# gillett-hernandez/rust-pathtracer

Hardware: AMD Instinct MI355X
Metric: Msamples/s (paths×spp/s) Cornell box 1024², max_bounces=8; 1/2/4/8 GPU (higher is better)
Workload: dtype f32

## Files before the change

### include/pt_api.h

```cpp
#ifndef PT_API_H
#define PT_API_H

#include <stddef.h>
#include <stdint.h>

#ifdef __cplusplus
extern "C" {
#endif

typedef int32_t pt_status;
enum {
    PT_OK = 0,
    PT_ERR_INVALID_ARGUMENT = 1,
    PT_ERR_NO_DEVICE = 2,
    PT_ERR_OUT_OF_MEMORY = 3,
    PT_ERR_UNSUPPORTED = 4,
    PT_ERR_DEVICE = 5
};

enum { PT_TAG_MATERIAL = 0, PT_TAG_LIGHT = 1, PT_TAG_CAMERA = 2 };
#define PT_MATERIAL_ID(tag, index) ((((uint32_t)(tag)) << 16) | ((uint32_t)(index) & 0xffffu))
#define PT_MATERIAL_TAG(id) (((id) >> 16) & 0x3u)
#define PT_MATERIAL_INDEX(id) ((id) & 0xffffu)
#define PT_MATERIAL_NONE 0xffffffffu
// ... 147 lines not shown
    uint32_t medium_aware;
} pt_render_desc;

enum {
    PT_TUNE_NO_LDS = 1u << 0,
    PT_TUNE_NO_CORE_LDS = 1u << 1,
    PT_TUNE_NO_PARK = 1u << 2,
    PT_TUNE_NO_LIVE_LIST = 1u << 3,
    PT_TUNE_EXACT_SLAB = 1u << 4,
    PT_TUNE_NO_CULL = 1u << 5,
    PT_TUNE_NO_SWEEP = 1u << 6,
    PT_TUNE_NO_MESH_SWEEP = 1u << 7,
    PT_TUNE_NO_KNOWN_LIGHT = 1u << 8,
    PT_TUNE_GENERAL_FORMS = 1u << 9,
    PT_TUNE_NO_FUSE = 1u << 10,
    PT_TUNE_NO_STAGE_TIMING = 1u << 11,
    PT_TUNE_MULTI_RCCL = 1u << 12,
    PT_TUNE_NO_ONE_LIGHT = 1u << 14,
    PT_TUNE_NO_CONVEX = 1u << 15,
    PT_TUNE_NO_MESH_SHORTCUTS = 1u << 16,
    PT_TUNE_NO_AXIS_SCAN = 1u << 13,
    PT_TUNE_NO_PASS_OVERLAP = 1u << 17,
    PT_TUNE_PASS_SKEW_SHIFT = 18,
    PT_TUNE_PASS_SKEW_MASK = 7
};
typedef struct pt_tuning {
    uint32_t flags;
    uint32_t batch_slots;
    uint32_t blocks_per_cu;
    uint32_t park_blocks_per_cu;
    int32_t park_dynamic;
    uint32_t shade_form;
    uint32_t lds_all_limit;
    uint32_t multi_virtual;
    uint32_t walk_evict_below;
    uint32_t walk_search_below;
    uint32_t park_block;
    uint32_t light_prepass_max;
    uint32_t top_evict_below;
    uint32_t group_evict_below;
    uint32_t reserved[2];
} pt_tuning;
void pt_tuning_default(pt_tuning* tuning);

typedef struct pt_profile {
    uint64_t bounce_rays, shadow_rays, light_rays, camera_rays, env_hits;
    double seconds;
// ... 73 lines not shown
```

### rust-pathtracer_amd/api.py

```python
import ctypes as C
import numpy as np

PT_OK = 0
PT_ERR_INVALID_ARGUMENT = 1
PT_ERR_UNSUPPORTED = 4
TAG_MATERIAL, TAG_LIGHT, TAG_CAMERA = 0, 1, 2
MATERIAL_NONE = 0xFFFFFFFF

CURVE_LINEAR, CURVE_TABULATED, CURVE_CAUCHY, CURVE_EXPONENTIAL, CURVE_INV_EXPONENTIAL, CURVE_BLACKBODY, CURVE_CONST = range(7)
INTERP_LINEAR, INTERP_NEAREST, INTERP_CUBIC = range(3)
TEXTURE1, TEXTURE4 = 1, 4
MATERIAL_LAMBERTIAN, MATERIAL_GGX, MATERIAL_DIFFUSE_LIGHT, MATERIAL_SHARP_LIGHT, MATERIAL_PASSTHROUGH = range(5)
MEDIUM_HG, MEDIUM_RAYLEIGH = range(2)
SIDED_FORWARD, SIDED_REVERSE, SIDED_DUAL = range(3)
SHAPE_RECT, SHAPE_SPHERE, SHAPE_DISK, SHAPE_MESH = range(4)
AXIS_X, AXIS_Y, AXIS_Z = range(3)
ENV_CONSTANT, ENV_SUN, ENV_HDR = range(3)


def material_id(tag, index):
    return ((tag & 3) << 16) | (index & 0xFFFF)


class Curve(C.Structure):
# ... 123 lines not shown
class ResidentDenoiseDesc(C.Structure):
    _fields_ = [("filter", DenoiseDesc), ("flags", C.c_uint32), ("reserved", C.c_uint32 * 3)]


class GuideChainDesc(C.Structure):
    _fields_ = [("max_chain", C.c_uint32), ("alpha_max", C.c_float), ("reserved", C.c_uint32 * 2)]


class Profile(C.Structure):
    _fields_ = [("bounce_rays", C.c_uint64), ("shadow_rays", C.c_uint64), ("light_rays", C.c_uint64),
                ("camera_rays", C.c_uint64), ("env_hits", C.c_uint64), ("seconds", C.c_double),
                ("kernel_seconds", C.c_double * 8), ("kernel_launches", C.c_uint64 * 8), ("stage_items", C.c_uint64 * 8)]

    def as_dict(self):
        return {"bounce_rays": self.bounce_rays, "shadow_rays": self.shadow_rays, "light_rays": self.light_rays,
                "camera_rays": self.camera_rays, "env_hits": self.env_hits, "seconds": self.seconds,
                "kernel_seconds": list(self.kernel_seconds), "kernel_launches": list(self.kernel_launches), "stage_items": list(self.stage_items)}


TUNE_NO_LDS, TUNE_NO_CORE_LDS, TUNE_NO_PARK, TUNE_NO_LIVE_LIST, TUNE_EXACT_SLAB, TUNE_NO_CULL, TUNE_NO_SWEEP, TUNE_NO_MESH_SWEEP, TUNE_NO_KNOWN_LIGHT, \
    TUNE_GENERAL_FORMS, TUNE_NO_FUSE, TUNE_NO_STAGE_TIMING, TUNE_MULTI_RCCL, TUNE_NO_AXIS_SCAN, TUNE_NO_ONE_LIGHT, TUNE_NO_CONVEX, TUNE_NO_MESH_SHORTCUTS, \
    TUNE_NO_PASS_OVERLAP = (1 << i for i in range(18))
TUNE_PASS_SKEW_SHIFT, TUNE_PASS_SKEW_MASK = 18, 7


class Tuning(C.Structure):
    _fields_ = [("flags", C.c_uint32), ("batch_slots", C.c_uint32), ("blocks_per_cu", C.c_uint32), ("park_blocks_per_cu", C.c_uint32),
                ("park_dynamic", C.c_int32), ("shade_form", C.c_uint32), ("lds_all_limit", C.c_uint32), ("multi_virtual", C.c_uint32),
                ("walk_evict_below", C.c_uint32), ("walk_search_below", C.c_uint32), ("park_block", C.c_uint32), ("light_prepass_max", C.c_uint32), ("top_evict_below", C.c_uint32), ("group_evict_below", C.c_uint32), ("reserved", C.c_uint32 * 2)]


class OutputDesc(C.Structure):
    _fields_ = [("width", C.c_uint32), ("height", C.c_uint32), ("tonemap", C.c_int32), ("luminance_only", C.c_int32),
                ("exposure", C.c_float), ("key_value", C.c_float), ("white_point", C.c_float), ("colorspace", C.c_int32),
                ("factor", C.c_float)]


TONEMAP_CLAMP, TONEMAP_REINHARD0, TONEMAP_REINHARD1 = range(3)
COLORSPACE_SRGB, COLORSPACE_REC709, COLORSPACE_REC2020 = range(3)
COMPARE_ABSOLUTE, COMPARE_RMSE, COMPARE_RELATIVE = range(3)


class CompareStats(C.Structure):
    _fields_ = [("linf", C.c_double * 4), ("mean_abs", C.c_double * 4), ("rmse", C.c_double), ("pixel_min", C.c_float),
                ("pixel_max", C.c_float), ("nonfinite", C.c_uint64)]

# ... 366 lines not shown
        handle = C.c_void_p()
        if tuning is not None:
            if library._scene_create_tuned is None:
                raise PtError(PT_ERR_UNSUPPORTED, "this library does not export %sscene_create_tuned (pt_tuning is the HIP engine's)" % library.prefix)
            library.check(library._scene_create_tuned(C.byref(desc), C.byref(tuning), C.byref(handle)))
        else:
            library.check(library._scene_create(C.byref(desc), C.byref(handle)))
        self.handle = handle

    def close(self):
        if self.handle:
            self.library._scene_destroy(self.handle)
            self.handle = None

    def __del__(self):
        try:
            self.close()
        except Exception:
            pass

    def uses_leaf_sweep(self):
        return bool(self.library._debug_scene_info(self.handle, 4))

    def render(self, rd):
        film = np.zeros((rd.height, rd.width, 4), dtype=np.float32)
        prof = Profile()
        self.library.check(self.library._render(self.handle, C.byref(rd), _fp(film), C.byref(prof)))
        return film, prof

    def render_spectral(self, rd, bins):
        if self.library._render_spectral is None:
            raise PtError(PT_ERR_UNSUPPORTED, "%s has no %srender_spectral entry" % (self.library.path, self.library.prefix))
        film = np.zeros((rd.height, rd.width, 4), dtype=np.float32)
        spectral = np.zeros((max(int(bins), 0), rd.height, rd.width), dtype=np.float32)
        sd = SpectralDesc(bins)
        prof = Profile()
        self.library.check(self.library._render_spectral(self.handle, C.byref(rd), C.byref(sd), _fp(film), _fp(spectral), C.byref(prof)))
        return film, spectral, prof

    def render_spectral_multi(self, rd, bins, device_mask=0):
        if self.library._render_spectral_multi is None:
            raise PtError(PT_ERR_UNSUPPORTED, "%s has no %srender_spectral_multi entry" % (self.library.path, self.library.prefix))
        film = np.zeros((rd.height, rd.width, 4), dtype=np.float32)
        spectral = np.zeros((max(int(bins), 0), rd.height, rd.width), dtype=np.float32)
        sd = SpectralDesc(bins)
        prof = Profile()
# ... 370 lines not shown
```

### rust-pathtracer_amd/csrc/pt_engine.hip

```cpp
#include <hip/hip_runtime.h>

#include <dlfcn.h>
#include <rccl/rccl.h>

#include <algorithm>
#include <chrono>
#include <condition_variable>
#include <functional>
#include <mutex>
#include <thread>
#include <cstdio>
#include <cstring>
#include <string>
#include <vector>

#include "pt_kernels.h"
#include "../../include/pt_adaptive.h"
#include "../../include/pt_spectral.h"
#include "../../include/pt_api.h"
#include "../../include/pt_debug.h"
#include "../../include/pt_denoise.h"
#include "../../include/pt_light_groups.h"
#include "pt_adaptive_select.h"
#include "pt_light_groups_launch.h"
// ... 256 lines not shown
    const float* film = nullptr; const uint32_t* counts = nullptr; const double* stats = nullptr; const float* spectral = nullptr;
    const float* denoised_bins = nullptr;
    GrowBuf load_film, load_counts, load_stats, load_spectral;
    GrowBuf guides, albedo, bin_albedo;
    GrowBuf color[2], geo, tent, flags, grad, bin_buf[2];
    GrowBuf den_film, den_var, den_bins;
    void end() { parts = 0; width = height = bins = 0; }
    void tidy() {
        if (!(parts & (PT_RESIDENT_BINS | PT_RESIDENT_BIN_ALBEDO | PT_RESIDENT_DENOISED_BINS))) bins = 0;
        if (!parts) width = height = 0;
    }
    struct pt_resident_info info() const { struct pt_resident_info i; i.width = width; i.height = height; i.bins = bins; i.parts = parts; return i; }
};

struct pt_scene {
    pth::HostScene host;
    pt_tuning tuning;
    MultiSetup multi;
    uint32_t* d_blob = nullptr;
    float* d_tex = nullptr;
    uint32_t blob_words = 0;
    int lds_mode = 0;
    uint32_t lacks = 0;
    int device = 0, num_cus = 0;
    DeviceBuffers buf;
    DeviceBuffers buf2;
    hipStream_t pass_stream = nullptr;
    std::vector<hipEvent_t> pass_deps;
    AdaptiveBuffers adaptive;
    std::vector<hipEvent_t> events, events2;
    GrowBuf film_cache;
    GrowBuf spectral_cache;
    bool spectral_valid = false;
    uint32_t spectral_width = 0, spectral_height = 0, spectral_bins = 0;
    std::vector<pt_scene*> spectral_shards;
    std::vector<uint32_t> shard_px;
    GrowBuf shard_packed;
    bool groups_valid = false;
    uint32_t groups_width = 0, groups_height = 0, groups_count = 0;
    GrowBuf group_films_cache, group_table, group_mix_cache;
    ResidentSet resident;
    GrowBuf assemble_staging, assemble_px;
    GrowBuf project_cache;
    std::vector<pt_scene*> replicas;
};

// ... 247 lines not shown
        if (sweep) for (uint32_t j = 0; j < bl[PT_HDR_SWEEP_COUNT]; ++j) walked += (bl[bl[PT_HDR_SWEEP_OFF] + j * PT_SWEEP_INST_WORDS + 1] & PT_SWEEP_WALKED) ? 1u : 0u;
        if (parked && walked == 1u) group_evict = tn.group_evict_below ? tn.group_evict_below : kGroupEvictBelow;
    }
    cfg.walk_policy = (tn.walk_evict_below ? tn.walk_evict_below : kWalkEvictBelow) | (tn.walk_search_below ? tn.walk_search_below : kWalkSearchBelow) << 8
                    | ((tn.flags & PT_TUNE_NO_AXIS_SCAN) ? 0u : PT_WALK_SCAN_AXIS)
                    | (top_evict <= 1u ? 0u : top_evict << 24)
                    | (group_evict <= 1u ? 0u : group_evict << 17);
    float env_prob; std::memcpy(&env_prob, &sc->host.blob[PT_HDR_ENV_PROB], sizeof env_prob);
    bool has_ggx = false;
    for (uint32_t i = 0; i < sc->host.blob[PT_HDR_MATERIAL_COUNT]; ++i) {
        const uint32_t kind = sc->host.blob[sc->host.blob[PT_HDR_MATERIAL_OFF] + i * PT_MAT_WORDS + PT_MAT_KIND];
        has_ggx = has_ggx || kind == PT_MATERIAL_GGX || kind == PT_MATERIAL_PASSTHROUGH;
    }
    const bool certs = !rd.medium_aware && (sc->host.blob[PT_HDR_FLAGS] & PT_FLAG_CONVEX) != 0u;
    const int shade_form = rd.medium_aware ? PT_SHADE_MEDIUM
                         : (env_prob != 0.0f || tn.shade_form == 2 || grouped) ? PT_SHADE_FULL : (has_ggx || certs || tn.shade_form == 1) ? PT_SHADE_NO_ENV : PT_SHADE_LEAN;
    cfg.certs = certs;
    uint32_t live_list = ((trav_form == PT_FORM_SWEEP || trav_form == PT_FORM_WALK || trav_form == PT_FORM_ANY) && shade_form == PT_SHADE_LEAN && !(tn.flags & PT_TUNE_NO_LIVE_LIST)) ? 1u : 0u;
#ifdef PT_EXPERIMENTS
    if (cfg.live_lists || getenv("PT_AMD_EXP_SHADOW")) live_list = 0u;
#endif
    const uint32_t camera_record = (shade_form == PT_SHADE_LEAN || shade_form == PT_SHADE_FULL || shade_form == PT_SHADE_MEDIUM) ? 1u : 0u;
    cfg.fuse = !(tn.flags & PT_TUNE_NO_FUSE) && (!hero || PT_FUSE_HERO) && trav_form == PT_FORM_SWEEP && shade_form == PT_SHADE_LEAN && (cfg.lacks & PT_SCENE_NO_XF) != 0;
    const uint32_t path_fields = hero ? Layout<4>::path_fields : (rd.medium_aware ? (uint32_t)PS_FIELDS + 2u : Layout<1>::path_fields);
    const uint32_t item_fields = hero ? Layout<4>::shadow_queue_fields(rd.light_samples ? rd.light_samples : 1) : Layout<1>::shadow_queue_fields(rd.light_samples ? rd.light_samples : 1);
    *plan = RenderPlan{capacity, grid, hero, park_block, park_block_extend, trav_form, shade_form, park_dynamic, park_big, cfg, live_list, camera_record,
                       path_fields, item_fields};
    return PT_OK;
}

pt_status read_profile(pt_scene* sc, const RenderPlan& plan, bool second_set, uint64_t camera_rays, uint64_t accumulated_pixels, const double* stage_ms, const uint64_t* stage_launches,
                       uint32_t rounds, double seconds, pt_profile* profile) {
    memset(profile, 0, sizeof(*profile));
    std::vector<unsigned long long> bs((size_t)plan.grid * BS_FIELDS);
    unsigned long long c[BS_FIELDS] = {0, 0, 0, 0, 0, 0};
    for (const unsigned long long* d_bs : {(const unsigned long long*)sc->buf.block_stats, (const unsigned long long*)(second_set ? sc->buf2.block_stats : nullptr)}) {
        if (!d_bs) continue;
        HIP_TRY(hipMemcpy(bs.data(), d_bs, sizeof(unsigned long long) * bs.size(), hipMemcpyDeviceToHost));
        for (int g = 0; g < plan.grid; ++g) for (int k = 0; k < BS_FIELDS; ++k) c[k] += bs[(size_t)g * BS_FIELDS + k];
    }
    profile->camera_rays = camera_rays;
    profile->bounce_rays = c[BS_VERTICES] + camera_rays;
    profile->shadow_rays = c[BS_SHADOW_RAYS];
    profile->env_hits = c[BS_ENV_HITS];
    profile->seconds = seconds;
    for (int i = 0; i < ST_COUNT; ++i) { profile->kernel_seconds[i] = stage_ms[i] * 1e-3; profile->kernel_launches[i] = stage_launches[i]; }
// ... 2 lines not shown
    profile->stage_items[6] = (uint64_t)plan.cfg.park_block;
    profile->stage_items[7] = plan.camera_record;
    profile->stage_items[5] = c[BS_MEDIUM_DROPS];
    profile->kernel_launches[5] = rounds;
    return PT_OK;
}

enum { DEP_FORK = 0, DEP_ACCUMULATED = 1, DEP_SKEW = 3, DEP_COUNT = 5 };

pt_status render_impl(pt_scene* sc, const pt_render_desc* rdp, float* d_film, hipStream_t stream, pt_profile* profile, const RenderJob& job) {
    if (!sc || !rdp || !d_film) return fail(PT_ERR_INVALID_ARGUMENT, "null argument");
    pt_render_desc rd;
    std::string err;
    if (!pth::normalize_render_desc(*rdp, (uint32_t)sc->host.cameras.size(), &rd, &err)) return fail(PT_ERR_INVALID_ARGUMENT, err);
    HIP_TRY(hipSetDevice(sc->device));

    const pt_adaptive_desc* adaptive = job.adaptive;
    std::vector<uint32_t> own_list;
    if (!job.shard_list) own_list = pth::shard_pixels(rd.width, rd.height, rd.tile_width, rd.tile_height, rd.shard_index, rd.shard_count);
    const std::vector<uint32_t>& pixels = job.shard_list ? *job.shard_list : own_list;
    RenderPlan plan;
    pt_status st = plan_render(sc, rd, job, pixels, stream, &plan);
    if (st != PT_OK) return st;
    const uint32_t capacity = plan.capacity;
    const int grid = plan.grid, trav_form = plan.trav_form, shade_form = plan.shade_form;
    const bool hero = plan.hero, park_dynamic = plan.park_dynamic;
    LaunchCfg cfg = plan.cfg;

#ifdef PT_EXPERIMENTS
    const bool need_hits = true;
#else
    const bool need_hits = !cfg.fuse;
#endif
    const uint32_t group_count = job.groups ? job.groups->group_count : 0u;
    st = ensure_buffers(sc, sc->buf, capacity, rd.light_samples, pixels.size() ? pixels.size() : 1, grid, (hero || rd.medium_aware) ? 4u : 1u, plan.park_block, need_hits, group_count);
    if (st != PT_OK) return st;
    DeviceBuffers& b = sc->buf;
    bool overlap = !(sc->tuning.flags & PT_TUNE_NO_PASS_OVERLAP);
    if (overlap) {
        const uint32_t n_px = (uint32_t)pixels.size();
        overlap = pth::plan_passes(n_px, rd.first_sample, adaptive ? rd.spp : rd.sample_count, capacity, rd.phase_samples).size() >= 2
               || (adaptive && adaptive->max_samples > rd.spp && pth::plan_passes(n_px, rd.spp, adaptive->step < adaptive->max_samples - rd.spp ? adaptive->step : adaptive->max_samples - rd.spp, capacity, rd.phase_samples).size() >= 2);
    }
    if (overlap) {
        bool ok = ensure_buffers(sc, sc->buf2, capacity, rd.light_samples, 0, grid, (hero || rd.medium_aware) ? 4u : 1u, plan.park_block, need_hits, group_count) == PT_OK;
        if (ok && !sc->pass_stream) ok = hipStreamCreateWithFlags(&sc->pass_stream, hipStreamNonBlocking) == hipSuccess;
// ... 255 lines not shown
    if (e == hipSuccess) e = hipMemcpy(sc->d_tex, sc->host.tex.data(), sizeof(float) * sc->host.tex.size(), hipMemcpyHostToDevice);
    if (e != hipSuccess) return fail(e == hipErrorOutOfMemory ? PT_ERR_OUT_OF_MEMORY : PT_ERR_DEVICE, hipGetErrorString(e));
    if (sc->lds_mode != PT_LDS_NONE) {
        e = allow_lds_extend(kParkBlobLimitBytes);
        if (e == hipSuccess) e = allow_lds_shade(kLdsBlobLimitBytes > PT_SHADE_LDS_BUDGET ? kLdsBlobLimitBytes : PT_SHADE_LDS_BUDGET);
        if (e == hipSuccess) e = allow_lds_shadow(kParkBlobLimitBytes + 16u * (64u * PT_MAX_LIGHT_SAMPLES + 64u) * 4u);
        if (e == hipSuccess) e = allow_lds_groups(kLdsBlobLimitBytes > PT_SHADE_LDS_BUDGET ? kLdsBlobLimitBytes : PT_SHADE_LDS_BUDGET, kLdsBlobLimitBytes);
        if (e != hipSuccess) return fail(PT_ERR_DEVICE, std::string("hipFuncSetAttribute(MaxDynamicSharedMemorySize): ") + hipGetErrorString(e));
    }
    return PT_OK;
}

void pt_tuning_default(pt_tuning* t) {
    if (!t) return;
    memset(t, 0, sizeof(*t));
    const struct { const char* name; uint32_t bit; } flags[] = {
        {"PT_AMD_NO_LDS", PT_TUNE_NO_LDS}, {"PT_AMD_NO_CORE_LDS", PT_TUNE_NO_CORE_LDS}, {"PT_AMD_NO_PARK", PT_TUNE_NO_PARK},
#ifdef PT_EXPERIMENTS
        {"PT_AMD_POOL", PT_TUNE_EXPERIMENT_POOL},
#endif

        {"PT_AMD_EXACT_SLAB", PT_TUNE_EXACT_SLAB}, {"PT_AMD_NO_CULL", PT_TUNE_NO_CULL}, {"PT_AMD_NO_SWEEP", PT_TUNE_NO_SWEEP}, {"PT_AMD_NO_MESH_SWEEP", PT_TUNE_NO_MESH_SWEEP},
        {"PT_AMD_NO_KNOWN_LIGHT", PT_TUNE_NO_KNOWN_LIGHT}, {"PT_AMD_GENERAL_FORMS", PT_TUNE_GENERAL_FORMS}, {"PT_AMD_NO_FUSE", PT_TUNE_NO_FUSE}, {"PT_AMD_MULTI_RCCL", PT_TUNE_MULTI_RCCL}, {"PT_AMD_NO_AXIS_SCAN", PT_TUNE_NO_AXIS_SCAN}, {"PT_AMD_NO_ONE_LIGHT", PT_TUNE_NO_ONE_LIGHT}, {"PT_AMD_NO_CONVEX", PT_TUNE_NO_CONVEX}, {"PT_AMD_NO_MESH_SHORTCUTS", PT_TUNE_NO_MESH_SHORTCUTS},
        {"PT_AMD_NO_LIVE_LIST", PT_TUNE_NO_LIVE_LIST}, {"PT_AMD_NO_PASS_OVERLAP", PT_TUNE_NO_PASS_OVERLAP},
    };
    for (const auto& f : flags) if (env_u32(f.name, 0)) t->flags |= f.bit;
    if (env_u32("PT_AMD_STAGE_TIMING", 1) == 0) t->flags |= PT_TUNE_NO_STAGE_TIMING;
    t->batch_slots = env_u32("PT_AMD_BATCH", 0);
    t->blocks_per_cu = env_u32("PT_AMD_BLOCKS_PER_CU", 0);
    t->park_blocks_per_cu = env_u32("PT_AMD_PARK_BLOCKS_PER_CU", 0);
    t->park_dynamic = getenv("PT_AMD_PARK_DYNAMIC") && *getenv("PT_AMD_PARK_DYNAMIC") ? (env_u32("PT_AMD_PARK_DYNAMIC", 0) != 0 ? 1 : 0) : -1;
    t->shade_form = env_u32("PT_AMD_SHADE_FORM", 0);
    t->lds_all_limit = env_u32("PT_AMD_LDS_ALL_LIMIT", 0);
    t->multi_virtual = env_u32("PT_AMD_MULTI_VIRTUAL", 0);
    t->walk_evict_below = env_u32("PT_AMD_WALK_EVICT_BELOW", 0);
    t->walk_search_below = env_u32("PT_AMD_WALK_SEARCH_BELOW", 0);
    t->park_block = env_u32("PT_AMD_PARK_BLOCK", 0);
    t->light_prepass_max = env_u32("PT_AMD_LIGHT_PREPASS_MAX", 0);
    t->top_evict_below = env_u32("PT_AMD_TOP_EVICT_BELOW", 0);
    t->group_evict_below = env_u32("PT_AMD_GROUP_EVICT_BELOW", 0);
    t->flags |= (env_u32("PT_AMD_PASS_SKEW", 0) & PT_TUNE_PASS_SKEW_MASK) << PT_TUNE_PASS_SKEW_SHIFT;
}

pt_status pt_scene_create(const pt_scene_desc* desc, pt_scene** out) {
    pt_tuning t;
    pt_tuning_default(&t);
    return pt_scene_create_tuned(desc, &t, out);
// ... 1082 lines not shown
}
pt_status pt_curve_eval(pt_scene* sc, uint32_t curve, size_t n, const float* lambda, float* value) {
    if (!sc || curve >= sc->host.curve_count) return fail(PT_ERR_INVALID_ARGUMENT, "bad curve");
    return probe_material(sc, 3, sc->host.curve_offsets[curve], n, lambda, nullptr, 0, nullptr, 0, value, nullptr, nullptr);
}

pt_status pt_debug_numerics(int which, size_t n, const float* x, const float* y, float* out) {
    pt_status st = ensure_device();
    if (st != PT_OK) return st;
    DevBuf dx, dy, dout;
    HIP_TRY(dx.alloc(4 * n)); HIP_TRY(dy.alloc(4 * n)); HIP_TRY(dout.alloc(4 * n));
    HIP_TRY(hipMemcpy(dx.p, x, 4 * n, hipMemcpyHostToDevice)); HIP_TRY(hipMemcpy(dy.p, y, 4 * n, hipMemcpyHostToDevice));
    hipLaunchKernelGGL(k_probe_numerics, dim3(256), dim3(kBlock), 0, 0, which, (uint32_t)n, dx.as<float>(), dy.as<float>(), dout.as<float>());
    HIP_TRY(hipGetLastError());
    HIP_TRY(hipDeviceSynchronize());
    HIP_TRY(hipMemcpy(out, dout.p, 4 * n, hipMemcpyDeviceToHost));
    return PT_OK;
}

uint32_t pt_debug_scene_info(pt_scene* sc, int what) {
    switch (what) { case 0: return sc->blob_words * 4; case 1: return (uint32_t)sc->lds_mode; case 2: return sc->host.light_count; case 3: return (uint32_t)sc->num_cus;
                    case 4: return sc->host.blob[PT_HDR_SWEEP_OFF] != 0 && !(sc->host.blob[PT_HDR_FLAGS] & PT_FLAG_NO_SWEEP) ? 1u : 0u;
                    case 7: return sc->host.blob[PT_HDR_CORE_WORDS] * 4;
                    case 8: return (uint32_t)(sc->host.tex.size() > 0xffffffffull ? 0xffffffffull : sc->host.tex.size());
                    default: return 0; }
}

}
```

### rust-pathtracer_amd/csrc/pt_kern_shade.hip

```cpp
#ifndef PT_SHADE_PART
#error "PT_SHADE_PART must be 0 (lean forms) or 1 (NO_ENV, FULL, medium)"
#endif
#include <cstdio>
#include <cstdlib>
#include "pt_kernels.h"

namespace ptk {

#define PT_GO(K, ...) go(c, K, __VA_ARGS__)
#define PT_BY_MODE(K, ...) do { if (c.lds_mode == PT_LDS_ALL) PT_GO(K(PT_LDS_ALL), __VA_ARGS__); else if (c.lds_mode == PT_LDS_CORE) PT_GO(K(PT_LDS_CORE), __VA_ARGS__); \
                                else PT_GO(K(PT_LDS_NONE), __VA_ARGS__); } while (0)
#define PT_NML PT_SCENE_NO_MESH_LIGHTS
#define K_SHADE_L(M) k_shade<M, PT_SHADE_NL, PT_SHADE_LEAN, PT_SCENE_NO_CERTS | PT_NML>
#define K_SHADE_LX(M) k_shade<M, PT_SHADE_NL, PT_SHADE_LEAN, PT_SCENE_NO_XF | PT_SCENE_NO_CERTS | PT_NML>
#define K_SHADE_FUSED k_shade<PT_LDS_ALL, PT_SHADE_NL, PT_SHADE_LEAN, PT_SCENE_NO_XF | PT_SCENE_NO_CERTS | PT_NML, PT_TRAV_SWEEP>
#define K_SHADE_N(M) k_shade<M, PT_SHADE_NL, PT_SHADE_NO_ENV, PT_SCENE_NO_CERTS | PT_NML>
#define K_SHADE_F(M) k_shade<M, PT_SHADE_NL, PT_SHADE_FULL, PT_SCENE_NO_CERTS | PT_NML>
#define K_SHADE_FE(M) k_shade<M, PT_SHADE_NL, PT_SHADE_FULL, PT_SCENE_NO_LIGHTS | PT_SCENE_NO_CERTS | PT_NML>
#define K_SHADE_NC(M) k_shade<M, PT_SHADE_NL, PT_SHADE_NO_ENV, PT_NML>
#define K_SHADE_FC(M) k_shade<M, PT_SHADE_NL, PT_SHADE_FULL, PT_NML>
#define K_SHADE_LM(M) k_shade<M, PT_SHADE_NL, PT_SHADE_LEAN, PT_SCENE_NO_CERTS>
#define K_SHADE_NM(M) k_shade<M, PT_SHADE_NL, PT_SHADE_NO_ENV, 0u>
#define K_SHADE_FM(M) k_shade<M, PT_SHADE_NL, PT_SHADE_FULL, 0u>
#define PT_ARGS sc.blob, sc.blob_words, sc.tex, rp, bounce, pixels, paths_in, hits, paths_out, shadow, energy, seg_cap, count_in, count_out, shadow_count, block_stats
#define PT_ARGS_FWD sc, rp, bounce, pixels, paths_in, hits, paths_out, shadow, energy, seg_cap, count_in, count_out, shadow_count, block_stats
#define PT_CAT2(a, b) a##b
#define PT_CAT(a, b) PT_CAT2(a, b)

#define PT_PARTNAME(base) PT_CAT(PT_CAT(PT_CAT(base, PT_SHADE_NL), _p), PT_SHADE_PART)
void PT_PARTNAME(launch_shade_nl)(const LaunchCfg& c, int form, const SceneArgs& sc, const RenderParams& rp, uint32_t bounce, const uint32_t* pixels, Queue paths_in,
                                          Queue hits, Queue paths_out, Queue shadow, float* energy, uint32_t seg_cap, const uint32_t* count_in, uint32_t* count_out,
                                          uint32_t* shadow_count, unsigned long long* block_stats) {
#if PT_SHADE_PART == 1
#if PT_SHADE_NL == 1
#define K_SHADE_M(M) k_shade_medium<M>
#define K_SHADE_MM(M) k_shade_medium<M, 0u>
    if (form == PT_SHADE_MEDIUM) { if (c.mesh_lights) PT_BY_MODE(K_SHADE_MM, PT_ARGS); else PT_BY_MODE(K_SHADE_M, PT_ARGS); return; }
#endif
    if (form == PT_SHADE_FULL) {
        LaunchCfg d = c; d.lds_bytes = ((c.lds_bytes + 15u) & ~15u) + sc.marg_bytes;
#define PT_GO_D(K, ...) go(d, K, __VA_ARGS__)
#define PT_BY_MODE_D(K, ...) do { if (c.lds_mode == PT_LDS_ALL) PT_GO_D(K(PT_LDS_ALL), __VA_ARGS__); else if (c.lds_mode == PT_LDS_CORE) PT_GO_D(K(PT_LDS_CORE), __VA_ARGS__); \
                                  else PT_GO_D(K(PT_LDS_NONE), __VA_ARGS__); } while (0)
        if (c.mesh_lights) PT_BY_MODE_D(K_SHADE_FM, PT_ARGS);
        else if (c.certs) PT_BY_MODE_D(K_SHADE_FC, PT_ARGS);
        else if ((c.lacks & PT_SCENE_NO_LIGHTS) && PT_SHADE_NL == 1) PT_BY_MODE_D(K_SHADE_FE, PT_ARGS);
        else PT_BY_MODE_D(K_SHADE_F, PT_ARGS);
    }
    else if (c.mesh_lights) PT_BY_MODE(K_SHADE_NM, PT_ARGS);
    else if (c.certs) PT_BY_MODE(K_SHADE_NC, PT_ARGS);
    else PT_BY_MODE(K_SHADE_N, PT_ARGS);
#else
    (void)form;
    if (c.mesh_lights) PT_BY_MODE(K_SHADE_LM, PT_ARGS);
    else if (c.fuse) PT_GO(K_SHADE_FUSED, PT_ARGS);
    else if (c.lacks & PT_SCENE_NO_XF) PT_BY_MODE(K_SHADE_LX, PT_ARGS);
    else PT_BY_MODE(K_SHADE_L, PT_ARGS);
#endif
    PT_TL_BUMP(c.stream);
}
hipError_t PT_PARTNAME(allow_lds_shade_nl)(uint32_t bytes) {
    hipError_t worst = hipSuccess;
    auto allow = [&](const void* k) { hipError_t e = hipFuncSetAttribute(k, hipFuncAttributeMaxDynamicSharedMemorySize, (int)bytes); if (e != hipSuccess) worst = e; };
#define PT_ALLOW_MODES(K) allow(reinterpret_cast<const void*>(K(PT_LDS_ALL))); allow(reinterpret_cast<const void*>(K(PT_LDS_CORE))); allow(reinterpret_cast<const void*>(K(PT_LDS_NONE)))
#if PT_SHADE_PART == 0
    allow(reinterpret_cast<const void*>(K_SHADE_FUSED));
    PT_ALLOW_MODES(K_SHADE_L); PT_ALLOW_MODES(K_SHADE_LX); PT_ALLOW_MODES(K_SHADE_LM);
#else
    PT_ALLOW_MODES(K_SHADE_N); PT_ALLOW_MODES(K_SHADE_F); PT_ALLOW_MODES(K_SHADE_NC); PT_ALLOW_MODES(K_SHADE_FC); PT_ALLOW_MODES(K_SHADE_NM); PT_ALLOW_MODES(K_SHADE_FM);
#if PT_SHADE_NL == 1
    PT_ALLOW_MODES(K_SHADE_FE);
    PT_ALLOW_MODES(K_SHADE_M); PT_ALLOW_MODES(K_SHADE_MM);
#endif
#endif
    return worst;
}

#if PT_SHADE_NL == 1 && PT_SHADE_PART == 0
#define PT_SHADE_SIG const LaunchCfg&, int, const SceneArgs&, const RenderParams&, uint32_t, const uint32_t*, Queue, Queue, Queue, Queue, float*, uint32_t, const uint32_t*, uint32_t*, uint32_t*, unsigned long long*
void launch_shade_nl1_p1(PT_SHADE_SIG); void launch_shade_nl4_p0(PT_SHADE_SIG); void launch_shade_nl4_p1(PT_SHADE_SIG);
hipError_t allow_lds_shade_nl1_p1(uint32_t); hipError_t allow_lds_shade_nl4_p0(uint32_t); hipError_t allow_lds_shade_nl4_p1(uint32_t);
void launch_shade(const LaunchCfg& c, int nl, int form, const SceneArgs& sc, const RenderParams& rp, uint32_t bounce, const uint32_t* pixels, Queue paths_in,
                  Queue hits, Queue paths_out, Queue shadow, float* energy, uint32_t seg_cap, const uint32_t* count_in, uint32_t* count_out,
                  uint32_t* shadow_count, unsigned long long* block_stats) {
    const bool lean = form == PT_SHADE_LEAN;
    if (c.certs && form == PT_SHADE_LEAN) { fprintf(stderr, "launch_shade: a scene with convex-body certificates takes the NO_ENV or FULL form\n"); abort(); }
    if ((rp.camera_record != 0u) != (form != PT_SHADE_NO_ENV)) { fprintf(stderr, "launch_shade: form %d launched with camera_record = %u\n", form, rp.camera_record); abort(); }
    if (nl == 4) { if (lean) launch_shade_nl4_p0(c, form, PT_ARGS_FWD); else launch_shade_nl4_p1(c, form, PT_ARGS_FWD); }
    else if (lean) launch_shade_nl1_p0(c, form, PT_ARGS_FWD); else launch_shade_nl1_p1(c, form, PT_ARGS_FWD);
// ... 13 lines not shown
```

### rust-pathtracer_amd/csrc/pt_kernels.h

```cpp
#ifndef PT_KERNELS_H
#define PT_KERNELS_H
#include <hip/hip_runtime.h>
#define PT_WAVE_KERNELS 1
#include "pt_launch.h"

namespace ptk {
using namespace ptd;

template <typename K, typename... Args>
inline void go(const LaunchCfg& c, K kernel, Args... args) { hipLaunchKernelGGL(kernel, dim3(c.grid), dim3(kBlock), c.lds_bytes, c.stream, args...); }
template <typename K, typename... Args>
inline void go_block(const LaunchCfg& c, int block, uint32_t lds_bytes, K kernel, Args... args) { hipLaunchKernelGGL(kernel, dim3(c.grid), dim3(block), lds_bytes, c.stream, args...); }

#ifndef PT_SHADE_WAVES
#define PT_SHADE_WAVES 4
#endif
#ifndef PT_MEDIUM_SPLIT
#define PT_MEDIUM_SPLIT 1
#endif
#ifndef PT_SHADE_MEDIUM_WAVES
#define PT_SHADE_MEDIUM_WAVES 3
#endif
#ifndef PT_SHADE4_WAVES
#define PT_SHADE4_WAVES 2
// ... 273 lines not shown
            }
            if (!(LACKS & PT_SCENE_NO_CERTS)) pv.slot &= ~PT_PATH_INSIDE_MARK;
            wants_item = shade_wants_item(s, rp, hit);
        }
        uint32_t ipos = base + shared_append(wants_item, &lds_counts[1]);
        constexpr bool kLiveList = FORM == PT_SHADE_LEAN;
        bool item_lives = false;
        ShadeOutT<NL> out;
        out.survives = false; out.has_item = false; out.vertex_pushed = false; out.env_hit = false; out.shadow_count = 0; out.add_energy = false; out.env_mask = 0;
        if (active) {
            uint32_t pixel = pixels[pv.slot % rp.chunk_pixels];
            out = stage_shade<NL, FORM == PT_SHADE_FULL, FORM != PT_SHADE_LEAN>(s, rp, bounce, pv, hit, pixel, [&](uint32_t l, const ShadowRayT<NL>& ray) { store_shadow_ray<NL>(shadow, ipos, l, ray); if (kLiveList) item_lives = item_lives || ray_is_live<NL>(ray); });
            if (wants_item) {
                float lam[NL]; lam[0] = pv.lambda;
                if (NL > 1) hero_lambdas<NL>(rp, pv.lambda, lam);
                qsu(shadow, Layout<NL>::sh_slot, ipos, pv.slot); qsu(shadow, Layout<NL>::sh_flags, ipos, out.env_mask);
                for (int k = 0; k < NL; ++k) qsf(shadow, Layout<NL>::sh_lambda + k, ipos, lam[k]);
                if (!out.has_item) clear_shadow_item<NL>(shadow, ipos, rp.light_samples);
            }
            if (out.add_energy) for (int k = 0; k < NL; ++k) energy[(size_t)k * rp.energy_stride + pv.slot] += out.energy_add[k];
        }
        uint32_t pos;
        if (kLiveList && rp.live_list) {
            uint32_t lpos;
            shared_append2(out.survives, &lds_counts[0], item_lives, &lds_counts[2], &pos, &lpos);
            pos += base;
            if (item_lives) qsu(shadow, Layout<NL>::shadow_live_field(rp.light_samples), base + lpos, ipos);
        } else pos = base + shared_append(out.survives, &lds_counts[0]);
        if (out.survives) store_path<NL>(paths_out, pos, out.next);
        st_vertices += out.vertex_pushed ? 1u : 0u; st_env += out.env_hit ? 1u : 0u; st_shadow += out.shadow_count;
#ifdef PT_TIMELINE
        tl_work += out.vertex_pushed ? 1u : 0u;
#endif
    }
    PT_TL_END(n);
    st_vertices = wave_reduce_add(st_vertices); st_shadow = wave_reduce_add(st_shadow); st_env = wave_reduce_add(st_env);
    if (lane_id() == 0) { atomicAdd(&lds_counts[4], st_vertices); atomicAdd(&lds_counts[5], st_shadow); atomicAdd(&lds_counts[6], st_env); }
    __syncthreads();
    if (threadIdx.x == 0) {
        count_out[blockIdx.x] = lds_counts[0]; shadow_count[blockIdx.x] = lds_counts[1]; shadow_count[gridDim.x + blockIdx.x] = lds_counts[2];
        unsigned long long* bs = block_stats + (size_t)blockIdx.x * BS_FIELDS;
        bs[BS_VERTICES] += lds_counts[4]; bs[BS_SHADOW_RAYS] += lds_counts[5]; bs[BS_ENV_HITS] += lds_counts[6];
        bs[BS_SEGMENTS] += n;
        bs[BS_ITEMS] += lds_counts[1];
    }
}
// ... 777 lines not shown
```

### rust-pathtracer_amd/csrc/pt_launch.h

```cpp
#ifndef PT_LAUNCH_H
#define PT_LAUNCH_H
#include <hip/hip_runtime.h>
#include "pt_stages.h"

namespace ptk {

enum { PT_LDS_NONE = 0, PT_LDS_ALL = 1, PT_LDS_CORE = 2 };
enum { PT_SHADE_LEAN = 0, PT_SHADE_NO_ENV = 1, PT_SHADE_FULL = 2, PT_SHADE_MEDIUM = 3 };
enum { PT_FORM_ANY = 0, PT_FORM_WALK = 1, PT_FORM_SWEEP = 2, PT_FORM_POOLED = 3, PT_FORM_PARKED = 4, PT_FORM_PARKED_WALK = 5 };
constexpr int kBlock = 256;
constexpr uint32_t kLdsBlobLimitBytes = 64 * 1024;
constexpr uint32_t kLdsAllLimitBytes = PT_BLOB_LDS_ALL_BYTES;
constexpr uint32_t kParkBlobLimitBytes = 72 * 1024;
constexpr uint32_t kParkCap = 512, kParkFields = 16;
constexpr uint32_t kLightPrepassMax = 16;
constexpr uint32_t kGroupEvictBelow = 32;
constexpr uint32_t kTopEvictBelow = 48;
constexpr uint32_t kWalkEvictBelow = 32, kWalkSearchBelow = 16;
enum { BS_VERTICES, BS_SHADOW_RAYS, BS_ENV_HITS, BS_SEGMENTS, BS_ITEMS, BS_MEDIUM_DROPS, BS_FIELDS };
#ifdef PT_EXPERIMENTS
uint32_t pool_lds_bytes();
#endif

struct LaunchCfg { int grid; uint32_t lds_bytes; hipStream_t stream; int lds_mode;
                   int dyn_grid = 0; uint32_t* unit_counter = nullptr;
                   uint32_t lacks = 0;
                   uint32_t walk_policy = 0;
                   int park_block = 0, park_block_extend = 0;
                   uint32_t park_blob_bytes = 0;
                   bool live_lists = false;
                   bool certs = false;
                   uint32_t path_marks = 0;
                   bool mesh_lights = false;
                   bool fuse = false; };
struct SceneArgs { const uint32_t* blob; uint32_t blob_words; const float* tex; uint32_t marg_bytes = 0;  };
inline uint32_t marginal_lds_bytes(const uint32_t* host_blob, uint32_t staged_bytes) {
    const uint32_t rows = host_blob[PT_HDR_IMAP_ROWS];
    if (host_blob[PT_HDR_ENV_KIND] != PT_ENV_HDR || rows == 0u || rows > PT_MARG_LDS_MAX_ROWS || host_blob[PT_HDR_IMAP_STRIDE] != 2u) return 0u;
    const uint32_t bytes = PT_MARG_LDS_BYTES(rows, host_blob[PT_HDR_IMAP_MARG_GUIDE] != 0u);
    return ((staged_bytes + 15u) & ~15u) + bytes <= PT_SHADE_LDS_BUDGET ? bytes : 0u;
}

void launch_extend(const LaunchCfg& c, int form, const SceneArgs& sc, ptd::Queue paths, ptd::Queue hits, uint32_t seg_cap, const uint32_t* count_in, uint32_t* park);
void launch_shade(const LaunchCfg& c, int nl, int form, const SceneArgs& sc, const ptd::RenderParams& rp, uint32_t bounce, const uint32_t* pixels, ptd::Queue paths_in,
                  ptd::Queue hits, ptd::Queue paths_out, ptd::Queue shadow, float* energy, uint32_t seg_cap, const uint32_t* count_in, uint32_t* count_out,
                  uint32_t* shadow_count, unsigned long long* block_stats);
void launch_shadow(const LaunchCfg& c, int form, int nl, bool env, const SceneArgs& sc, uint32_t light_samples, ptd::Queue shadow, float* energy, uint32_t energy_stride,
                   uint32_t seg_cap, const uint32_t* count_in, uint32_t* park, ptd::Queue idle_hits);
void launch_probe_intersect(const LaunchCfg& c, const SceneArgs& sc, uint32_t n, const float* o, const float* d, pt_hit* out);
hipError_t allow_lds_extend(uint32_t bytes);
hipError_t allow_lds_shade(uint32_t bytes);
hipError_t allow_lds_shadow(uint32_t bytes);

}
#endif
```

Measured before the change: 2472.

## Add vertex-fill fused shade kernel that compacts hit lanes through LDS carry buffer

Adds a new fused traverse+shade kernel that parks valid hits in a per-wave LDS carry buffer and only runs the expensive shading once a full wave of 64 hits is gathered. Misses are handled immediately and leftovers are flushed at the end. The goal is less SIMD divergence in shading caused by rays that miss or terminate. In exchange it uses extra LDS, which may lower occupancy, and adds ballot/popcount bookkeeping and extra rounds. It is on by default whenever the fused path is chosen and the LDS budget allows, and can be turned off with a tuning flag.

```diff
diff --git a/include/pt_api.h b/include/pt_api.h
--- a/include/pt_api.h
+++ b/include/pt_api.h
@@ -193,7 +193,8 @@
     PT_TUNE_NO_AXIS_SCAN = 1u << 13,
     PT_TUNE_NO_PASS_OVERLAP = 1u << 17,
     PT_TUNE_PASS_SKEW_SHIFT = 18,
-    PT_TUNE_PASS_SKEW_MASK = 7
+    PT_TUNE_PASS_SKEW_MASK = 7,
+    PT_TUNE_NO_VERTEX_FILL = 1u << 21
 };
 typedef struct pt_tuning {
     uint32_t flags;
diff --git a/rust-pathtracer_amd/api.py b/rust-pathtracer_amd/api.py
--- a/rust-pathtracer_amd/api.py
+++ b/rust-pathtracer_amd/api.py
@@ -169,6 +169,7 @@
     TUNE_GENERAL_FORMS, TUNE_NO_FUSE, TUNE_NO_STAGE_TIMING, TUNE_MULTI_RCCL, TUNE_NO_AXIS_SCAN, TUNE_NO_ONE_LIGHT, TUNE_NO_CONVEX, TUNE_NO_MESH_SHORTCUTS, \
     TUNE_NO_PASS_OVERLAP = (1 << i for i in range(18))
 TUNE_PASS_SKEW_SHIFT, TUNE_PASS_SKEW_MASK = 18, 7
+TUNE_NO_VERTEX_FILL = 1 << 21
 
 
 class Tuning(C.Structure):
@@ -581,6 +582,9 @@
     def uses_leaf_sweep(self):
         return bool(self.library._debug_scene_info(self.handle, 4))
 
+    def uses_vertex_fill(self):
+        return bool(self.library._debug_scene_info(self.handle, 9))
+
     def render(self, rd):
         film = np.zeros((rd.height, rd.width, 4), dtype=np.float32)
         prof = Profile()
diff --git a/rust-pathtracer_amd/csrc/pt_engine.hip b/rust-pathtracer_amd/csrc/pt_engine.hip
--- a/rust-pathtracer_amd/csrc/pt_engine.hip
+++ b/rust-pathtracer_amd/csrc/pt_engine.hip
@@ -302,6 +302,7 @@
     uint32_t blob_words = 0;
     int lds_mode = 0;
     uint32_t lacks = 0;
+    bool planned_vertex_fill = false;
     int device = 0, num_cus = 0;
     DeviceBuffers buf;
     DeviceBuffers buf2;
@@ -595,6 +596,7 @@
 #endif
     const uint32_t camera_record = (shade_form == PT_SHADE_LEAN || shade_form == PT_SHADE_FULL || shade_form == PT_SHADE_MEDIUM) ? 1u : 0u;
     cfg.fuse = !(tn.flags & PT_TUNE_NO_FUSE) && (!hero || PT_FUSE_HERO) && trav_form == PT_FORM_SWEEP && shade_form == PT_SHADE_LEAN && (cfg.lacks & PT_SCENE_NO_XF) != 0;
+    cfg.vertex_fill = cfg.fuse && !(tn.flags & PT_TUNE_NO_VERTEX_FILL) && vf_fits(lds_bytes, (uint32_t)kBlock, PT_SHADE_LDS_BUDGET);
     const uint32_t path_fields = hero ? Layout<4>::path_fields : (rd.medium_aware ? (uint32_t)PS_FIELDS + 2u : Layout<1>::path_fields);
     const uint32_t item_fields = hero ? Layout<4>::shadow_queue_fields(rd.light_samples ? rd.light_samples : 1) : Layout<1>::shadow_queue_fields(rd.light_samples ? rd.light_samples : 1);
     *plan = RenderPlan{capacity, grid, hero, park_block, park_block_extend, trav_form, shade_form, park_dynamic, park_big, cfg, live_list, camera_record,
@@ -643,6 +645,7 @@
     RenderPlan plan;
     pt_status st = plan_render(sc, rd, job, pixels, stream, &plan);
     if (st != PT_OK) return st;
+    sc->planned_vertex_fill = plan.cfg.vertex_fill;
     const uint32_t capacity = plan.capacity;
     const int grid = plan.grid, trav_form = plan.trav_form, shade_form = plan.shade_form;
     const bool hero = plan.hero, park_dynamic = plan.park_dynamic;
@@ -944,7 +947,7 @@
 
         {"PT_AMD_EXACT_SLAB", PT_TUNE_EXACT_SLAB}, {"PT_AMD_NO_CULL", PT_TUNE_NO_CULL}, {"PT_AMD_NO_SWEEP", PT_TUNE_NO_SWEEP}, {"PT_AMD_NO_MESH_SWEEP", PT_TUNE_NO_MESH_SWEEP},
         {"PT_AMD_NO_KNOWN_LIGHT", PT_TUNE_NO_KNOWN_LIGHT}, {"PT_AMD_GENERAL_FORMS", PT_TUNE_GENERAL_FORMS}, {"PT_AMD_NO_FUSE", PT_TUNE_NO_FUSE}, {"PT_AMD_MULTI_RCCL", PT_TUNE_MULTI_RCCL}, {"PT_AMD_NO_AXIS_SCAN", PT_TUNE_NO_AXIS_SCAN}, {"PT_AMD_NO_ONE_LIGHT", PT_TUNE_NO_ONE_LIGHT}, {"PT_AMD_NO_CONVEX", PT_TUNE_NO_CONVEX}, {"PT_AMD_NO_MESH_SHORTCUTS", PT_TUNE_NO_MESH_SHORTCUTS},
-        {"PT_AMD_NO_LIVE_LIST", PT_TUNE_NO_LIVE_LIST}, {"PT_AMD_NO_PASS_OVERLAP", PT_TUNE_NO_PASS_OVERLAP},
+        {"PT_AMD_NO_LIVE_LIST", PT_TUNE_NO_LIVE_LIST}, {"PT_AMD_NO_PASS_OVERLAP", PT_TUNE_NO_PASS_OVERLAP}, {"PT_AMD_NO_VERTEX_FILL", PT_TUNE_NO_VERTEX_FILL},
     };
     for (const auto& f : flags) if (env_u32(f.name, 0)) t->flags |= f.bit;
     if (env_u32("PT_AMD_STAGE_TIMING", 1) == 0) t->flags |= PT_TUNE_NO_STAGE_TIMING;
@@ -2073,6 +2076,7 @@
     switch (what) { case 0: return sc->blob_words * 4; case 1: return (uint32_t)sc->lds_mode; case 2: return sc->host.light_count; case 3: return (uint32_t)sc->num_cus;
                     case 4: return sc->host.blob[PT_HDR_SWEEP_OFF] != 0 && !(sc->host.blob[PT_HDR_FLAGS] & PT_FLAG_NO_SWEEP) ? 1u : 0u;
                     case 7: return sc->host.blob[PT_HDR_CORE_WORDS] * 4;
+                    case 9: return sc->planned_vertex_fill ? 1u : 0u;
                     case 8: return (uint32_t)(sc->host.tex.size() > 0xffffffffull ? 0xffffffffull : sc->host.tex.size());
                     default: return 0; }
 }
diff --git a/rust-pathtracer_amd/csrc/pt_kern_shade.hip b/rust-pathtracer_amd/csrc/pt_kern_shade.hip
--- a/rust-pathtracer_amd/csrc/pt_kern_shade.hip
+++ b/rust-pathtracer_amd/csrc/pt_kern_shade.hip
@@ -14,6 +14,7 @@
 #define K_SHADE_L(M) k_shade<M, PT_SHADE_NL, PT_SHADE_LEAN, PT_SCENE_NO_CERTS | PT_NML>
 #define K_SHADE_LX(M) k_shade<M, PT_SHADE_NL, PT_SHADE_LEAN, PT_SCENE_NO_XF | PT_SCENE_NO_CERTS | PT_NML>
 #define K_SHADE_FUSED k_shade<PT_LDS_ALL, PT_SHADE_NL, PT_SHADE_LEAN, PT_SCENE_NO_XF | PT_SCENE_NO_CERTS | PT_NML, PT_TRAV_SWEEP>
+#define K_SHADE_FILL k_shade_fill<PT_SHADE_NL, PT_SCENE_NO_XF | PT_SCENE_NO_CERTS | PT_NML>
 #define K_SHADE_N(M) k_shade<M, PT_SHADE_NL, PT_SHADE_NO_ENV, PT_SCENE_NO_CERTS | PT_NML>
 #define K_SHADE_F(M) k_shade<M, PT_SHADE_NL, PT_SHADE_FULL, PT_SCENE_NO_CERTS | PT_NML>
 #define K_SHADE_FE(M) k_shade<M, PT_SHADE_NL, PT_SHADE_FULL, PT_SCENE_NO_LIGHTS | PT_SCENE_NO_CERTS | PT_NML>
@@ -53,6 +54,7 @@
 #else
     (void)form;
     if (c.mesh_lights) PT_BY_MODE(K_SHADE_LM, PT_ARGS);
+    else if (c.fuse && c.vertex_fill) PT_GO(K_SHADE_FILL, PT_ARGS);
     else if (c.fuse) PT_GO(K_SHADE_FUSED, PT_ARGS);
     else if (c.lacks & PT_SCENE_NO_XF) PT_BY_MODE(K_SHADE_LX, PT_ARGS);
     else PT_BY_MODE(K_SHADE_L, PT_ARGS);
@@ -64,7 +66,7 @@
     auto allow = [&](const void* k) { hipError_t e = hipFuncSetAttribute(k, hipFuncAttributeMaxDynamicSharedMemorySize, (int)bytes); if (e != hipSuccess) worst = e; };
 #define PT_ALLOW_MODES(K) allow(reinterpret_cast<const void*>(K(PT_LDS_ALL))); allow(reinterpret_cast<const void*>(K(PT_LDS_CORE))); allow(reinterpret_cast<const void*>(K(PT_LDS_NONE)))
 #if PT_SHADE_PART == 0
-    allow(reinterpret_cast<const void*>(K_SHADE_FUSED));
+    allow(reinterpret_cast<const void*>(K_SHADE_FUSED)); allow(reinterpret_cast<const void*>(K_SHADE_FILL));
     PT_ALLOW_MODES(K_SHADE_L); PT_ALLOW_MODES(K_SHADE_LX); PT_ALLOW_MODES(K_SHADE_LM);
 #else
     PT_ALLOW_MODES(K_SHADE_N); PT_ALLOW_MODES(K_SHADE_F); PT_ALLOW_MODES(K_SHADE_NC); PT_ALLOW_MODES(K_SHADE_FC); PT_ALLOW_MODES(K_SHADE_NM); PT_ALLOW_MODES(K_SHADE_FM);
diff --git a/rust-pathtracer_amd/csrc/pt_kernels.h b/rust-pathtracer_amd/csrc/pt_kernels.h
--- a/rust-pathtracer_amd/csrc/pt_kernels.h
+++ b/rust-pathtracer_amd/csrc/pt_kernels.h
@@ -319,6 +319,130 @@
         }
         uint32_t pos;
         if (kLiveList && rp.live_list) {
+            uint32_t lpos;
+            shared_append2(out.survives, &lds_counts[0], item_lives, &lds_counts[2], &pos, &lpos);
+            pos += base;
+            if (item_lives) qsu(shadow, Layout<NL>::shadow_live_field(rp.light_samples), base + lpos, ipos);
+        } else pos = base + shared_append(out.survives, &lds_counts[0]);
+        if (out.survives) store_path<NL>(paths_out, pos, out.next);
+        st_vertices += out.vertex_pushed ? 1u : 0u; st_env += out.env_hit ? 1u : 0u; st_shadow += out.shadow_count;
+#ifdef PT_TIMELINE
+        tl_work += out.vertex_pushed ? 1u : 0u;
+#endif
+    }
+    PT_TL_END(n);
+    st_vertices = wave_reduce_add(st_vertices); st_shadow = wave_reduce_add(st_shadow); st_env = wave_reduce_add(st_env);
+    if (lane_id() == 0) { atomicAdd(&lds_counts[4], st_vertices); atomicAdd(&lds_counts[5], st_shadow); atomicAdd(&lds_counts[6], st_env); }
+    __syncthreads();
+    if (threadIdx.x == 0) {
+        count_out[blockIdx.x] = lds_counts[0]; shadow_count[blockIdx.x] = lds_counts[1]; shadow_count[gridDim.x + blockIdx.x] = lds_counts[2];
+        unsigned long long* bs = block_stats + (size_t)blockIdx.x * BS_FIELDS;
+        bs[BS_VERTICES] += lds_counts[4]; bs[BS_SHADOW_RAYS] += lds_counts[5]; bs[BS_ENV_HITS] += lds_counts[6];
+        bs[BS_SEGMENTS] += n;
+        bs[BS_ITEMS] += lds_counts[1];
+    }
+}
+
+template <int NL, uint32_t LACKS>
+__global__ void __launch_bounds__(kBlock) __attribute__((amdgpu_waves_per_eu(NL == 1 ? PT_FUSED_WAVES : PT_FUSED4_WAVES)))
+k_shade_fill(const uint32_t* __restrict__ blob, uint32_t blob_words, const float* __restrict__ tex, RenderParams rp, uint32_t bounce, const uint32_t* __restrict__ pixels,
+             Queue paths_in, Queue hits, Queue paths_out, Queue shadow, float* __restrict__ energy, uint32_t seg_cap, const uint32_t* __restrict__ count_in,
+             uint32_t* __restrict__ count_out, uint32_t* __restrict__ shadow_count, unsigned long long* __restrict__ block_stats) {
+    static_assert((LACKS & PT_SCENE_NO_CERTS) != 0u && (LACKS & PT_SCENE_NO_XF) != 0u, "the fused form's scenes: no certificates, no transforms");
+    extern __shared__ __align__(16) uint32_t lds[];
+    __shared__ uint32_t lds_counts[16];
+    __shared__ uint32_t carry[kBlock / VF_WAVE * VF_WAVE_WORDS];
+    (void)hits;
+    if (PT_EMPTY_SEGMENT_EXIT && count_in[blockIdx.x] == 0u) {
+        if (threadIdx.x == 0) { count_out[blockIdx.x] = 0u; shadow_count[blockIdx.x] = 0u; shadow_count[gridDim.x + blockIdx.x] = 0u; }
+        return;
+    }
+    if (threadIdx.x < 16) lds_counts[threadIdx.x] = 0;
+    SceneView s = stage_scene<PT_LDS_ALL, LACKS>(blob, blob_words, tex, lds);
+    const uint32_t base = blockIdx.x * seg_cap, n = count_in[blockIdx.x];
+    uint32_t st_vertices = 0, st_shadow = 0, st_env = 0;
+    const uint32_t rounds = (n + blockDim.x - 1) / blockDim.x;
+    uint32_t* my_carry = carry + (threadIdx.x >> 6) * VF_WAVE_WORDS;
+    uint32_t carried = 0;
+    auto carry_store = [&](uint32_t e, const Hit& h, uint32_t item) {
+        my_carry[vf_word(0, e)] = __float_as_uint(h.t);
+        my_carry[vf_word(1, e)] = __float_as_uint(h.p.x); my_carry[vf_word(2, e)] = __float_as_uint(h.p.y); my_carry[vf_word(3, e)] = __float_as_uint(h.p.z);
+        my_carry[vf_word(4, e)] = __float_as_uint(h.n.x); my_carry[vf_word(5, e)] = __float_as_uint(h.n.y); my_carry[vf_word(6, e)] = __float_as_uint(h.n.z);
+        my_carry[vf_word(7, e)] = __float_as_uint(h.u); my_carry[vf_word(8, e)] = __float_as_uint(h.v);
+        my_carry[vf_word(9, e)] = h.material; my_carry[vf_word(10, e)] = h.instance; my_carry[vf_word(VF_INDEX, e)] = item;
+    };
+    auto carry_load = [&](uint32_t e, Hit* h, uint32_t* item) {
+        h->t = __uint_as_float(my_carry[vf_word(0, e)]);
+        h->p = f3(__uint_as_float(my_carry[vf_word(1, e)]), __uint_as_float(my_carry[vf_word(2, e)]), __uint_as_float(my_carry[vf_word(3, e)]));
+        h->n = f3(__uint_as_float(my_carry[vf_word(4, e)]), __uint_as_float(my_carry[vf_word(5, e)]), __uint_as_float(my_carry[vf_word(6, e)]));
+        h->u = __uint_as_float(my_carry[vf_word(7, e)]); h->v = __uint_as_float(my_carry[vf_word(8, e)]);
+        h->material = my_carry[vf_word(9, e)]; h->instance = my_carry[vf_word(10, e)]; *item = my_carry[vf_word(VF_INDEX, e)];
+        h->valid = true;
+    };
+    static_assert(VF_HIT_WORDS == 11 && VF_INDEX == 11, "carry_store / carry_load: a Hit's eleven words and the item's index");
+    PT_TL_BEGIN();
+    for (uint32_t r = 0;;) {
+        uint32_t i = 0;
+        Hit hit; hit.valid = false;
+        if (r < rounds) {
+            const uint32_t j = r * blockDim.x + threadIdx.x;
+            ++r;
+            const bool fresh = j < n;
+            i = base + j;
+            if (fresh) {
+                const F3 o = f3(qf(paths_in, PS_OX, i), qf(paths_in, PS_OY, i), qf(paths_in, PS_OZ, i));
+                const F3 d = f3(qf(paths_in, PS_DX, i), qf(paths_in, PS_DY, i), qf(paths_in, PS_DZ, i));
+                world_hit<PT_TRAV_SWEEP>(s, o, d, &hit);
+            }
+            if (fresh && !hit.valid) {
+                const PathVertexT<NL> pv = load_path<NL>(paths_in, i, bounce == 0u);
+                Hit none; none.valid = false;
+                const ShadeOutT<NL> out = stage_shade<NL, false, false>(s, rp, bounce, pv, none, pixels[pv.slot % rp.chunk_pixels], [](uint32_t, const ShadowRayT<NL>&) {});
+                if (out.add_energy) for (int k = 0; k < NL; ++k) energy[(size_t)k * rp.energy_stride + pv.slot] += out.energy_add[k];
+                st_vertices += out.vertex_pushed ? 1u : 0u; st_env += out.env_hit ? 1u : 0u;
+            }
+            const unsigned long long m = __ballot(hit.valid);
+            const VfTurn t = vf_turn(carried, (uint32_t)__popcll(m));
+            const uint32_t rank = (uint32_t)__popcll(m & ((1ull << lane_id()) - 1ull));
+            if (!t.shade) {
+                if (hit.valid) carry_store(vf_push_entry(carried, rank), hit, i);
+                carried = t.carried;
+                __builtin_amdgcn_wave_barrier();
+                continue;
+            }
+            if (!hit.valid) carry_load(vf_pull_entry(carried, lane_id() - rank), &hit, &i);
+            carried = t.carried;
+            __builtin_amdgcn_wave_barrier();
+        } else if (carried > 0u) {
+            const uint32_t take = vf_flush(carried);
+            carried = 0u;
+            if (lane_id() < take) carry_load(lane_id(), &hit, &i);
+        } else break;
+        const bool active = hit.valid;
+        PathVertexT<NL> pv;
+        bool wants_item = false;
+        if (active) {
+            pv = load_path<NL>(paths_in, i, bounce == 0u);
+            wants_item = shade_wants_item(s, rp, hit);
+        }
+        uint32_t ipos = base + shared_append(wants_item, &lds_counts[1]);
+        bool item_lives = false;
+        ShadeOutT<NL> out;
+        out.survives = false; out.has_item = false; out.vertex_pushed = false; out.env_hit = false; out.shadow_count = 0; out.add_energy = false; out.env_mask = 0;
+        if (active) {
+            uint32_t pixel = pixels[pv.slot % rp.chunk_pixels];
+            out = stage_shade<NL, false, false>(s, rp, bounce, pv, hit, pixel, [&](uint32_t l, const ShadowRayT<NL>& ray) { store_shadow_ray<NL>(shadow, ipos, l, ray); item_lives = item_lives || ray_is_live<NL>(ray); });
+            if (wants_item) {
+                float lam[NL]; lam[0] = pv.lambda;
+                if (NL > 1) hero_lambdas<NL>(rp, pv.lambda, lam);
+                qsu(shadow, Layout<NL>::sh_slot, ipos, pv.slot); qsu(shadow, Layout<NL>::sh_flags, ipos, out.env_mask);
+                for (int k = 0; k < NL; ++k) qsf(shadow, Layout<NL>::sh_lambda + k, ipos, lam[k]);
+                if (!out.has_item) clear_shadow_item<NL>(shadow, ipos, rp.light_samples);
+            }
+            if (out.add_energy) for (int k = 0; k < NL; ++k) energy[(size_t)k * rp.energy_stride + pv.slot] += out.energy_add[k];
+        }
+        uint32_t pos;
+        if (rp.live_list) {
             uint32_t lpos;
             shared_append2(out.survives, &lds_counts[0], item_lives, &lds_counts[2], &pos, &lpos);
             pos += base;
diff --git a/rust-pathtracer_amd/csrc/pt_launch.h b/rust-pathtracer_amd/csrc/pt_launch.h
--- a/rust-pathtracer_amd/csrc/pt_launch.h
+++ b/rust-pathtracer_amd/csrc/pt_launch.h
@@ -2,6 +2,7 @@
 #define PT_LAUNCH_H
 #include <hip/hip_runtime.h>
 #include "pt_stages.h"
+#include "pt_vertex_fill_rules.h"
 
 namespace ptk {
 
@@ -32,7 +33,8 @@
                    bool certs = false;
                    uint32_t path_marks = 0;
                    bool mesh_lights = false;
-                   bool fuse = false; };
+                   bool fuse = false;
+                   bool vertex_fill = false; };
 struct SceneArgs { const uint32_t* blob; uint32_t blob_words; const float* tex; uint32_t marg_bytes = 0;  };
 inline uint32_t marginal_lds_bytes(const uint32_t* host_blob, uint32_t staged_bytes) {
     const uint32_t rows = host_blob[PT_HDR_IMAP_ROWS];
diff --git a/rust-pathtracer_amd/csrc/pt_vertex_fill_rules.h b/rust-pathtracer_amd/csrc/pt_vertex_fill_rules.h
--- /dev/null
+++ b/rust-pathtracer_amd/csrc/pt_vertex_fill_rules.h
@@ -0,0 +1,33 @@
+#ifndef PT_VERTEX_FILL_RULES_H
+#define PT_VERTEX_FILL_RULES_H
+#include <stdint.h>
+#include "../../include/pt_numerics.h"
+
+namespace ptd {
+
+constexpr uint32_t VF_WAVE = 64;
+constexpr uint32_t VF_CAP = VF_WAVE - 1;
+constexpr uint32_t VF_HIT_WORDS = 11, VF_INDEX = VF_HIT_WORDS, VF_FIELDS = VF_HIT_WORDS + 1;
+constexpr uint32_t VF_WAVE_WORDS = VF_FIELDS * VF_WAVE;
+PT_HD uint32_t vf_word(uint32_t field, uint32_t entry) { return field * VF_WAVE + entry; }
+PT_HD uint32_t vf_lds_bytes(uint32_t threads) { return threads / VF_WAVE * VF_WAVE_WORDS * 4u; }
+PT_HD bool vf_fits(uint32_t staged_bytes, uint32_t threads, uint32_t budget) { return ((staged_bytes + 15u) & ~15u) + vf_lds_bytes(threads) <= budget; }
+
+struct VfTurn {
+    bool shade;
+    uint32_t pull;
+    uint32_t carried;
+};
+PT_HD VfTurn vf_turn(uint32_t carried, uint32_t hits) {
+    VfTurn t;
+    t.shade = carried + hits >= VF_WAVE;
+    t.pull = t.shade ? VF_WAVE - hits : 0u;
+    t.carried = t.shade ? carried - t.pull : carried + hits;
+    return t;
+}
+PT_HD uint32_t vf_pull_entry(uint32_t carried, uint32_t rank) { return carried - 1u - rank; }
+PT_HD uint32_t vf_push_entry(uint32_t carried, uint32_t rank) { return carried + rank; }
+PT_HD uint32_t vf_flush(uint32_t carried) { return carried; }
+
+}
+#endif
```

Measured after the change: 2491, median of 6. About the same (+0.8%).
